# terry19850829Home/kafkastreams-cep

Hardware: AMD Instinct MI355X
Metric: events/sec (whole node), 3-stage A->B->C over 1M keys; achieved HBM GB/s (higher is better)
Workload: dtype int32; 1 GPU; C2: 3-stage strict A->B->C, processor mode; events_per_gpu=100000000, keys_per_gpu=1000000, matches_per_gpu=1531088, matches_total=1531088, parallelism=1 GPU, kernels=built-in, nfa_kernel=auto

## Files before the change

kafkastreams-cep_amd/csrc/compile.cpp:

```cpp
#include <math.h>
#include <string.h>

#include <algorithm>
#include <limits>

#include "kcep_internal.h"
#include "../../include/kcep.h"

namespace kcep {
namespace {

struct Reader {
  const uint8_t* p;
  size_t n, i = 0;
  bool bad = false;
  bool need(size_t k) {
    if (i + k > n) bad = true;
    return !bad;
  }
  template <class T>
  T get() {
    T v{};
    if (need(sizeof(T))) { memcpy(&v, p + i, sizeof(T)); i += sizeof(T); }
    return v;
// ... 335 lines not shown
  if (S.coltype == T_I32) {
    for (auto& b : bi) b = std::max<int64_t>(b, INT32_MIN);
    bi.erase(std::remove_if(bi.begin(), bi.end(), [](int64_t b) { return b > INT32_MAX; }), bi.end());
  }
  for (auto& b : tb) b = std::max<int64_t>(b, INT32_MIN);
  tb.erase(std::remove_if(tb.begin(), tb.end(), [](int64_t b) { return b > INT32_MAX; }), tb.end());
  uniq(bi); uniq(bf); uniq(tb);
  const int nb = int(isf ? bf.size() : bi.size());
  if (nb > 15 || tb.size() > 3) return false;
  S.nbp = nb;
  S.ntbp = int(tb.size());
  for (int i = 0; i < nb; i++) { if (isf) S.bpf[i] = bf[i]; else S.bpi[i] = bi[i]; }
  for (size_t i = 0; i < tb.size(); i++) S.tbp[i] = int32_t(tb[i]);
  memset(S.table, 0, sizeof S.table);
  memset(S.nan_mask, 0, sizeof S.nan_mask);
  for (int it = 0; it <= S.ntbp; it++) {
    const int64_t trep = it == 0 ? (S.ntbp ? int64_t(S.tbp[0]) - 1 : 0) : int64_t(S.tbp[it - 1]);
    for (int iv = 0; iv <= nb; iv++) {
      int64_t vi = 0;
      double vf = 0;
      if (isf) vf = iv == 0 ? -INFINITY : bf[iv - 1];
      else vi = iv == 0 ? (nb ? bi[0] - (bi[0] > IMIN ? 1 : 0) : 0) : bi[iv - 1];
      uint8_t m = 0;
      for (int s = 0; s < STENCIL_MAX_K; s++) m |= uint8_t(stage_accepts(S, s, isf, vi, vf, trep)) << s;
      S.table[it * 16 + iv] = m;
    }
    uint8_t m = 0;
    for (int s = 0; s < STENCIL_MAX_K; s++) m |= uint8_t(stage_accepts(S, s, isf, 0, NAN, trep)) << s;
    S.nan_mask[it] = m;
  }
  S.lut_n = 0;
  S.lut_lo = 0;
  memset(S.lut, 0, sizeof S.lut);
  if (!isf && S.ntbp == 0 && nb >= 6 && bi.back() - bi.front() < int64_t(sizeof S.lut)) {
    S.lut_lo = bi.front();
    S.lut_n = int32_t(bi.back() - bi.front() + 1);
    for (int r = 0, iv = 0; r < S.lut_n; r++) {
      while (iv < nb && bi[iv] <= S.lut_lo + r) iv++;
      S.lut[r] = S.table[iv];
    }
  }
  return true;
}

bool stencil_shape(const Program& P, uint32_t& opt, std::string& why) {
  auto no = [&](const char* w) { why = w; return false; };
  const int k = int(P.pats.size());
  if (k > STENCIL_MAX_K) return no("more than 8 stages");
  opt = 0;
  for (int i = 0; i < k; i++) {
    const auto& p = P.pats[i];
    if (p.strategy != S_STRICT) return no("non-strict selection strategy");
    if (p.one_or_more || p.times > 1) return no("quantifier");
    if (p.optional) {
      if (i == 0) return no("optional first stage");
      opt |= 1u << i;
    }
    if (!p.folds.empty()) return no("fold");
    for (int j = 0; j < i; j++)
      if (P.pats[j].name_id == p.name_id) return no("duplicate stage names");
  }
  if (opt && k > CHAIN_MAX_K) return no("optional stages in a pattern of more than 4 stages");
  return true;
}

void put_slot(StencilProgram& S, int slot, const DNF& d) {
  S.nterms[slot] = int(d.size());
  S.pslots |= 1 << slot;
  for (size_t t = 0; t < d.size(); t++) {
    const Term& tm = d[t];
    S.vi[slot][t] = tm.has_v ? StencilAtomI{tm.v.lo, tm.v.hi} : StencilAtomI{IMIN, IMAX};
    S.vf[slot][t] = tm.has_v ? StencilAtomF{tm.v.dlo, tm.v.dhi} : StencilAtomF{-INFINITY, INFINITY};
    S.tp[slot][t] = tm.has_t ? StencilAtomI{tm.t.lo, tm.t.hi} : StencilAtomI{IMIN, IMAX};
// ... 344 lines not shown
  memset(&M, 0, sizeof M);
  CodeGen cg;
  cg.names = &P.names;
  const char* unfit = nullptr;
  auto slot = [&](int s, const ExprP& pred) {
    if (!unfit) unfit = mask_unfit(pred);
    if (unfit || !event_only(pred)) return;
    mask_reads(pred, M);
    M.pslots |= 1 << s;
    M.pc[s] = cg.emit(pred);
  };
  for (int i = 0; i < k; i++) {
    const auto& p = P.pats[i];
    S.name[i] = p.name_id;
    slot(i, p.topic >= 0 ? mk(OP_AND, mk_topic(p.topic), p.pred) : p.pred);
    if (opt >> i & 1) slot(CHAIN_MAX_K + i, P.pats[i + 1].pred);
  }
  if (unfit) return no(unfit);
  if (!cg.ok) return no(cg.why);
  if (cg.maxdepth > NFA_STACK) return no("expression nests deeper than the device operand stack");
  if (cg.code.size() > size_t(NFA_MAX_CODE)) return no("predicate code too large");
  M.ncols = int32_t(P.coltypes.size());
  for (size_t c = 0; c < P.coltypes.size(); c++) M.coltype[c] = P.coltypes[c];
  M.ncode = int32_t(cg.code.size());
  memcpy(M.code, cg.code.data(), cg.code.size() * sizeof(int32_t));
  S.k = k;
  S.chain = opt ? 1 : 0;
  S.optmask = int32_t(opt);
  S.pslots = M.pslots;
  S.col = -1;
  S.coltype = T_I32;
  S.lut_lo = 0;
  S.lut_n = 256;
  for (int m = 0; m < 256; m++) S.lut[m] = uint8_t(m);
  P.mask_ok = true;
  P.mask_why.clear();
}

}

int lower_general(Program& P, std::string& why) {
  DevProgram& D = P.dev;
  memset(&D, 0, sizeof D);
  if (P.stages.size() > size_t(NFA_MAX_STAGES)) { why = "too many stages"; return CEP_E_UNSUPPORTED; }
  if (P.states.size() > size_t(NFA_MAX_STATES)) { why = "too many states"; return CEP_E_UNSUPPORTED; }
  if (P.coltypes.size() > 16) { why = "too many columns"; return CEP_E_UNSUPPORTED; }
  D.nstages = int32_t(P.stages.size());
  D.begin = P.begin;
  D.nstates = int32_t(P.states.size());
  D.ncols = int32_t(P.coltypes.size());
  {
    std::vector<int> depth(P.stages.size(), 1);
    for (int id = 0; id < int(P.stages.size()); id++)
      for (auto& e : P.stages[id].edges)
        if ((e.op == E_PROCEED || e.op == E_SKIP_PROCEED) && e.target >= 0)
          depth[id] = std::max(depth[id], depth[e.target] + 1);
    int m = 0;
    for (int d : depth) m = std::max(m, d);
    D.maxdepth = m + 1;
    if (D.maxdepth > NFA_MAX_FRAMES) { why = "PROCEED chain deeper than the device frame stack"; return CEP_E_UNSUPPORTED; }
  }
  for (size_t c = 0; c < P.coltypes.size(); c++) D.coltype[c] = P.coltypes[c];
  D.ndefined = int32_t(P.defined_states.size());
  for (size_t i = 0; i < P.defined_states.size(); i++) D.defined[i] = P.defined_states[i];
  std::vector<std::pair<int, int>> slots;
  CodeGen cg;
  cg.names = &P.names;
// ... 132 lines not shown
```

kafkastreams-cep_amd/csrc/follow.hip:

```cpp
#include "stencil_kernel.h"

namespace kcep {

static_assert(FOLLOW_TILE == ST_TILE, "follow_bits takes the stencil kernels' tile: one chunk per thread");
static_assert(FOLLOW_TILE == 64 * 64, "a tile is 64 bitmap words: one second-level word");

typedef unsigned long long u64;

int64_t follow_tiles(int64_t n) { return (std::max<int64_t>(n, 1) + FOLLOW_TILE - 1) / FOLLOW_TILE; }

struct FollowMaps {
  const u64* bits;
  const u64* sum;
  int64_t wpl;
  int64_t nt;
  int64_t n;
  int32_t k;
  uint32_t next;
};

__device__ __forceinline__ int64_t next_set(const u64* __restrict__ plane, const u64* __restrict__ sum, int64_t from,
                                            int64_t limit) {
  if (from >= limit) return limit;
  int64_t w = from >> 6;
// ... 8 lines not shown
    sx = sum[sw];
  }
  w = sw * 64 + __builtin_ctzll(sx);
  return w * 64 + __builtin_ctzll(plane[w]);
}

__device__ __forceinline__ int64_t follow_walk(const FollowMaps& M, int64_t j0, int32_t* __restrict__ row) {
  const int64_t E = next_set(M.bits + M.k * M.wpl, M.sum + M.k * M.nt, j0 + 1, M.n);
  const int64_t end = E < M.n ? E : M.n;
  int64_t p = j0;
  if (row) row[0] = int32_t(j0);
  for (int s = 1; s < M.k; s++) {
    const u64* plane = M.bits + s * M.wpl;
    p++;
    if (M.next >> s & 1) {
      p = next_set(plane, M.sum + s * M.nt, p, end);
      if (p >= end) return -1;
    } else if (p >= end || !(plane[p >> 6] >> (p & 63) & 1)) {
      return -1;
    }
    if (row) row[s] = int32_t(p);
  }
  return p;
}

template <class VT, bool TOPIC>
__global__ __launch_bounds__(ST_THREADS) void follow_bits(const int32_t* __restrict__ key, const VT* __restrict__ val,
                                                         const int32_t* __restrict__ topic, int64_t n,
                                                         const StencilProgram* __restrict__ P, int k,
                                                         u64* __restrict__ bits, u64* __restrict__ sum, int64_t wpl,
                                                         int64_t nt, int64_t* __restrict__ tile_starts) {
  __shared__ __attribute__((aligned(16))) uint8_t s_mask[ST_TILE];
  __shared__ __attribute__((aligned(16))) uint8_t s_ks[ST_TILE];
  __shared__ uint8_t s_tab[64];
  __shared__ uint8_t s_lut[256];
  __shared__ uint8_t s_nan[4];
  __shared__ uint32_t s_part[STENCIL_MAX_K + 1][ST_THREADS / 64];
  __shared__ int32_t s_cnt[ST_THREADS / 64];

  const int tid = threadIdx.x;
  const int lane = tid & 63, wid = tid >> 6;
  if (tid < 64) s_tab[tid] = P->table[tid];
  s_lut[tid] = P->lut[tid];
  if (tid < 4) s_nan[tid] = P->nan_mask[tid];
  const int64_t tile = blockIdx.x;
  const int64_t base = tile * ST_TILE;

  Chunk<VT, TOPIC> cur;
  load_chunk<VT, TOPIC>(cur, key, val, topic, base, n, tid);
  int32_t before[ST_EPT / 4];
#pragma unroll
  for (int q = 0; q < ST_EPT / 4; q++) {
    const int64_t g = base + q * (ST_THREADS * 4) + tid * 4;
    before[q] = 0;
    if (lane == 0 && g > 0 && g < n) before[q] = key[g - 1];
  }
  __syncthreads();
  uint32_t packed[4];
  masks_of_chunk<VT, TOPIC>(cur, P, s_tab, s_nan, packed, s_lut);
#pragma unroll
  for (int q = 0; q < ST_EPT / 4; q++) {
    const int local = q * (ST_THREADS * 4) + tid * 4;
    const int64_t g = base + local;
    const v4i kv = cur.k[q];
    int32_t kp = __shfl_up(kv[3], 1);
    if (lane == 0) kp = before[q];
    uint32_t ks = uint32_t(g == 0 || kp != kv[0]) | (uint32_t(kv[1] != kv[0]) << 8) | (uint32_t(kv[2] != kv[1]) << 16) |
                  (uint32_t(kv[3] != kv[2]) << 24);
    uint32_t w = packed[q];
    const int64_t left = n - g;
    if (left < 4) {
      const uint32_t keep = left <= 0 ? 0u : (0xFFFFFFFFu >> (8 * (4 - left)));
      w &= keep;
      ks &= keep;
    }
    *reinterpret_cast<uint32_t*>(&s_mask[local]) = w;
    *reinterpret_cast<uint32_t*>(&s_ks[local]) = ks;
  }
  __syncthreads();
  u64 mine[STENCIL_MAX_K + 1];
#pragma unroll
  for (int s = 0; s <= STENCIL_MAX_K; s++) mine[s] = 0;
  for (int i = 0; i < 16; i++) {
    const int r = (wid * 16 + i) * 64 + lane;
    const uint32_t m = s_mask[r];
    const u64 bk = __ballot(s_ks[r] != 0);
    if (lane == i) mine[STENCIL_MAX_K] = bk;
#pragma unroll
    for (int s = 0; s < STENCIL_MAX_K; s++) {
      if (s < k) {
        const u64 bs = __ballot((m >> s & 1) != 0);
        if (lane == i) mine[s] = bs;
// ... 126 lines not shown
```

kafkastreams-cep_amd/csrc/kcep_internal.h:

```cpp
#pragma once
#include <hip/hip_runtime_api.h>
#include <stdint.h>
#include "kcep_dev.h"

#include <memory>
#include <string>
#include <vector>

namespace kcep {

struct Expr {
  uint8_t op = 0, t = 0, ct = 0;
  int32_t i32 = 0;
  int64_t i64 = 0;
  double f64 = 0;
  int col = 0, name = 0;
  std::string sname;
  std::shared_ptr<Expr> a, b;
};
using ExprP = std::shared_ptr<Expr>;

struct Fold {
  int state;
  uint8_t type;
// ... 4 lines not shown
  std::string name;
  int name_id = 0, level = 0;
  uint8_t strategy = S_STRICT;
  int32_t topic = -1;
  uint8_t one_or_more = 0, optional = 0;
  int32_t times = 1;
  int64_t window_ms = -1;
  ExprP pred;
  std::vector<Fold> folds;
};

struct EdgeDef {
  uint8_t op;
  ExprP pred;
  int target;
};

struct StageDef {
  int id, name;
  uint8_t type;
  int64_t window_ms;
  int pattern;
  std::vector<EdgeDef> edges;
};

constexpr int STENCIL_MAX_K = 8;
constexpr int STENCIL_MAX_TERMS = 6;
constexpr int STENCIL_MAX_ATOMS = 2;

struct StencilAtomI { int64_t lo, hi; };
struct StencilAtomF { double lo, hi; };

constexpr int CHAIN_MAX_K = 4;
struct StencilProgram {
  int32_t k;
  int32_t col;
  int32_t coltype;
  int32_t use_topic;
  int32_t chain;
  int32_t optmask;
  int32_t pslots;
  int32_t nterms[STENCIL_MAX_K];
  int32_t hasv[STENCIL_MAX_K][STENCIL_MAX_TERMS];
  StencilAtomI vi[STENCIL_MAX_K][STENCIL_MAX_TERMS];
  StencilAtomF vf[STENCIL_MAX_K][STENCIL_MAX_TERMS];
  StencilAtomI tp[STENCIL_MAX_K][STENCIL_MAX_TERMS];
  int32_t name[STENCIL_MAX_K];
  int32_t nbp;
  int32_t ntbp;
  int64_t bpi[15];
  double bpf[15];
  int32_t tbp[3];
  uint8_t table[64];
  uint8_t nan_mask[4];
  int64_t lut_lo;
  int32_t lut_n;
  uint8_t lut[256];
};

struct Program {
  std::vector<uint8_t> coltypes;
  std::vector<PatternDef> pats;
  std::vector<StageDef> stages;
  std::vector<std::string> names;
  std::vector<std::string> states;
  std::vector<int> defined_states;
  int begin = -1;
  bool general_ok = false;
  std::string general_why;
  DevProgram dev{};
  bool stencil_ok = false;
  std::string stencil_why;
  bool runs_ok = false;
  bool has_seq = false;
  std::string runs_why;
  StencilProgram stencil{};
  bool mask_ok = false;
  std::string mask_why;
  StencilProgram mask_stencil{};
  MaskProgram mask_prog{};
  bool follow_ok = false;
  std::string follow_why;
  StencilProgram follow{};
  uint32_t follow_next = 0;
};

struct HaloHdr {
  int32_t stamp[2];
  int32_t claim;
  uint8_t cnt[2];
// ... 27 lines not shown
```

kafkastreams-cep_amd/csrc/stencil_kernel.h:

```cpp
#pragma once
#include <hip/hip_runtime.h>
#include <stdint.h>

#include <type_traits>

#include "launch.h"

namespace kcep {

constexpr int ST_THREADS = 256;
constexpr int ST_EPT = 16;
constexpr int ST_TILE = ST_THREADS * ST_EPT;
constexpr int ST_SUB = 4;
inline int stencil_sub(int64_t ntiles) { return ntiles >= int64_t(ST_SUB) * 2048 ? ST_SUB : 1; }

typedef int v4i __attribute__((ext_vector_type(4)));
typedef long long v2l __attribute__((ext_vector_type(2)));
__device__ __forceinline__ v4i ld_nt4(const void* p) { return __builtin_nontemporal_load(reinterpret_cast<const v4i*>(p)); }
__device__ __forceinline__ v2l ld_nt2(const void* p) { return __builtin_nontemporal_load(reinterpret_cast<const v2l*>(p)); }

__device__ __forceinline__ int kpos(int rp) { return rp + 4 * (rp >> 4); }
constexpr int ST_KWORDS = (ST_TILE + 16) + 4 * ((ST_TILE + 16) >> 4) + 16;

template <class VT>
// ... 31 lines not shown
  for (int q = 0; q < ST_EPT / 4; q++) {
    const int64_t g = base + q * STRIDE + tid * 4;
    if (g + 3 < n) {
      if constexpr (KEYS) c.k[q] = ld_nt4(key + g);
      if constexpr (sizeof(VT) == 4) {
        c.v[q].a = ld_nt4(val + g);
      } else {
        c.v[q].a = ld_nt2(val + g);
        c.v[q].b = ld_nt2(val + g + 2);
      }
      if constexpr (TOPIC) c.t[q] = ld_nt4(topic + g);
    } else {
      const int64_t g0 = g < n ? g : n - 1, g1 = g + 1 < n ? g + 1 : n - 1;
      const int64_t g2 = g + 2 < n ? g + 2 : n - 1, g3 = g + 3 < n ? g + 3 : n - 1;
      if constexpr (KEYS) c.k[q] = v4i{key[g0], key[g1], key[g2], key[g3]};
      if constexpr (sizeof(VT) == 4) {
        c.v[q].a = v4i{__builtin_bit_cast(int32_t, val[g0]), __builtin_bit_cast(int32_t, val[g1]),
                       __builtin_bit_cast(int32_t, val[g2]), __builtin_bit_cast(int32_t, val[g3])};
      } else {
        c.v[q].a = v2l{__builtin_bit_cast(long long, val[g0]), __builtin_bit_cast(long long, val[g1])};
        c.v[q].b = v2l{__builtin_bit_cast(long long, val[g2]), __builtin_bit_cast(long long, val[g3])};
      }
      if constexpr (TOPIC) c.t[q] = v4i{topic[g0], topic[g1], topic[g2], topic[g3]};
    }
  }
}

template <class VT>
__device__ __forceinline__ VT bp_at(const StencilProgram* __restrict__ P, int b) {
  if constexpr (std::is_same<VT, double>::value) return P->bpf[b];
  else return VT(P->bpi[b]);
}

template <class VT, bool TOPIC>
__device__ __forceinline__ void masks_of_chunk(const Chunk<VT, TOPIC>& c, const StencilProgram* __restrict__ P,
                                               const uint8_t* s_tab, const uint8_t* s_nan, uint32_t (&packed)[4],
                                               const uint8_t* s_lut) {
  if constexpr (!TOPIC && !std::is_same<VT, double>::value) {
    const int32_t lut_n = P->lut_n;
    if (lut_n > 0) {
      const int64_t lo = P->lut_lo;
      const uint32_t below = s_tab[0], above = s_tab[P->nbp];
#pragma unroll
      for (int q = 0; q < 4; q++) {
        uint32_t w = 0;
#pragma unroll
        for (int i = 0; i < 4; i++) {
          const int64_t dv = int64_t(vget<VT>(c.v[q], i)) - lo;
          const uint32_t m = dv < 0 ? below : dv >= lut_n ? above : uint32_t(s_lut[dv]);
          w |= m << (8 * i);
        }
        packed[q] = w;
      }
      return;
    }
  }
  int iv[ST_EPT], it[ST_EPT];
#pragma unroll
  for (int e = 0; e < ST_EPT; e++) { iv[e] = 0; it[e] = 0; }
  const int nbp = P->nbp;
  for (int b = 0; b < nbp; b++) {
    const VT bp = bp_at<VT>(P, b);
#pragma unroll
    for (int e = 0; e < ST_EPT; e++) iv[e] += bp <= vget<VT>(c.v[e >> 2], e & 3) ? 1 : 0;
  }
  if constexpr (TOPIC) {
    const int ntbp = P->ntbp;
    for (int b = 0; b < ntbp; b++) {
      const int32_t tb = P->tbp[b];
#pragma unroll
      for (int e = 0; e < ST_EPT; e++) {
        const int32_t tv = c.t[e >> 2][e & 3];
        it[e] += tb <= tv ? 1 : 0;
      }
    }
  }
#pragma unroll
  for (int q = 0; q < 4; q++) {
    uint32_t w = 0;
#pragma unroll
    for (int i = 0; i < 4; i++) {
      const int e = 4 * q + i;
      uint32_t m = s_tab[it[e] * 16 + iv[e]];
      if constexpr (std::is_same<VT, double>::value) {
        const double v = vget<VT>(c.v[q], i);
        if (v != v) m = s_nan[it[e]];
      }
      w |= m << (8 * i);
    }
    packed[q] = w;
  }
}

template <class VT, bool TOPIC>
__device__ __forceinline__ uint32_t mask_of(const StencilProgram* __restrict__ P, const uint8_t* s_tab,
                                            const uint8_t* s_nan, VT v, int32_t t, const uint8_t* s_lut) {
  if constexpr (!TOPIC && !std::is_same<VT, double>::value) {
    const int32_t lut_n = P->lut_n;
    if (lut_n > 0) {
      const int64_t dv = int64_t(v) - P->lut_lo;
      return dv < 0 ? s_tab[0] : dv >= lut_n ? s_tab[P->nbp] : s_lut[dv];
    }
  }
  int iv = 0, it = 0;
  for (int b = 0; b < P->nbp; b++) iv += bp_at<VT>(P, b) <= v ? 1 : 0;
  if constexpr (TOPIC)
    for (int b = 0; b < P->ntbp; b++) it += P->tbp[b] <= t ? 1 : 0;
  if constexpr (std::is_same<VT, double>::value)
    if (v != v) return s_nan[it];
  return s_tab[it * 16 + iv];
}

template <int K>
struct ChainWin {
  uint32_t b[K];
  uint32_t s[K];
  uint32_t same;
};

__device__ __forceinline__ uint32_t byte_bits(uint64_t m, int i) {
  return uint32_t((((m >> i) & 0x0101010101010101ull) * 0x0102040810204080ull) >> 56);
}

template <int K>
__device__ __forceinline__ ChainWin<K> chain_window(const int32_t (&wk)[24], const uint64_t (&m8)[3], uint32_t opt) {
  ChainWin<K> c;
#pragma unroll
  for (int i = 0; i < K; i++) { c.b[i] = 0; c.s[i] = 0; }
  c.same = 0;
#pragma unroll
  for (int q = 0; q < 3; q++) {
#pragma unroll
    for (int i = 0; i < K; i++) {
      c.b[i] |= byte_bits(m8[q], i) << (8 * q);
      c.s[i] |= byte_bits(m8[q], CHAIN_MAX_K + i) << (8 * q);
    }
  }
#pragma unroll
  for (int w = 1; w < 24; w++) c.same |= uint32_t(wk[w] == wk[w - 1]) << w;
#pragma unroll
  for (int i = 0; i < K; i++)
    if (!((opt >> i) & 1)) c.s[i] = 0;
  return c;
// ... 119 lines not shown
        if ((m >> stage) & 1) { cm |= 1u << stage; stage++; alive = true; break; }
        if (((opt >> stage) & 1) && ((m >> (CHAIN_MAX_K + stage)) & 1)) { stage++; continue; }
        break;
      }
      if (!alive) break;
      if (stage == K) { done = v == d; break; }
    }
    if (done) { res |= 1u << d; cms[d] = cm; }
  }
  return res;
}

__device__ __forceinline__ int32_t stencil_row(int32_t rj, uint32_t a, int s, int k, bool chain, bool carry) {
  if (chain) {
    const uint32_t d = a & 3u, cm = (a >> 2) & 15u;
    const int ho = int(a >> 6);
    const int rel = -int32_t(d) + __popc(cm & ((1u << s) - 1));
    if (!((cm >> s) & 1)) return -1;
    if (carry && ho != 3 && rel < -ho) return -(1 + (-ho - rel));
    return rj + rel;
  }
  const int need = carry ? int(a) : 0;
  return s < need ? -(1 + (need - s)) : rj - (k - 1) + s;
}

template <int K, class VT, bool TOPIC, bool CHAIN, bool CARRY, int SUB>
__global__ __launch_bounds__(ST_THREADS) void stencil_kernel(
    const int32_t* __restrict__ key, const VT* __restrict__ val, const int32_t* __restrict__ topic, int64_t n,
    const StencilProgram* __restrict__ P, int32_t* __restrict__ out, int64_t* __restrict__ tile_count,
    int64_t ntiles, StencilCarry C) {
  __shared__ __attribute__((aligned(16))) int32_t s_key[ST_KWORDS];
  __shared__ __attribute__((aligned(16))) uint8_t s_mask[ST_TILE + 16];
  __shared__ int32_t s_wsum[SUB][ST_THREADS / 64];
  __shared__ uint8_t s_tab[64];
  __shared__ uint8_t s_lut[256];
  __shared__ uint8_t s_nan[4];
  __shared__ uint32_t s_super;

  const int tid = threadIdx.x;
  const int lane = tid & 63, wid = tid >> 6;
  if (tid == 0) s_super = blockIdx.x;
  if (tid < 64) s_tab[tid] = P->table[tid];
  s_lut[tid] = P->lut[tid];
  if (tid < 4) s_nan[tid] = P->nan_mask[tid];
  __syncthreads();
  const int64_t tile0 = int64_t(s_super) * SUB;
  const int ntl = int(ntiles - tile0 < SUB ? ntiles - tile0 : SUB);

  Chunk<VT, TOPIC> cur;
  load_chunk<VT, TOPIC>(cur, key, val, topic, tile0 * ST_TILE, n, tid);
  int32_t h_key = INT32_MIN;
  uint32_t h_mask = 0;
  VT h_val{};
  int32_t h_top = 0;
  const bool halo_lane = tid >= 16 - (K - 1) && tid < 16;
  const bool h_first = halo_lane && tile0 * ST_TILE - 16 + tid >= 0;
  if (h_first) {
    const int64_t g = tile0 * ST_TILE - 16 + tid;
    h_key = key[g];
    h_val = val[g];
    if constexpr (TOPIC) h_top = topic[g];
  }

  uint32_t hits[SUB];
  uint64_t bneed[CARRY ? SUB : 1];
  int excl[SUB], total[SUB];
  uint32_t wpk[CHAIN ? SUB : 1][2 * K], wsame[CHAIN ? SUB : 1];
  uint32_t hb[CHAIN && CARRY ? SUB : 1];
  const uint32_t opt = CHAIN ? uint32_t(P->optmask) : 0u;

#pragma unroll
  for (int j = 0; j < SUB; j++) {
    hits[j] = 0; excl[j] = 0; total[j] = 0;
    if (j < ntl) {
      const int64_t tile = tile0 + j;
      const int64_t base = tile * ST_TILE;
      const int lb = ST_EPT * tid + 8;
// ... 16 lines not shown
        ck[24] = tid + 1 < ST_THREADS ? s_key[kpos(lb + 24)] : (base + ST_TILE < n ? key[base + ST_TILE] : INT32_MIN);
        const int64_t g0 = base + tid * ST_EPT;
        uint32_t starts = 0;
#pragma unroll
        for (int i = 0; i < ST_EPT; i++) {
          const int32_t kj = ck[8 + i];
          bool full = true;
#pragma unroll
          for (int t = 1; t < K; t++) full = full && ck[8 + i - t] == kj;
          const bool live = g0 + i < n;
          bnd |= uint32_t(live && !full) << i;
          endm |= uint32_t(live && (ck[9 + i] != kj || g0 + i + 1 >= n)) << i;
          starts |= uint32_t(ck[7 + i] != kj) << i;
        }
        starts &= bnd;
        todo = bnd | endm;
        if (todo) {
          ka = ck[8 + __ffs(todo) - 1];
          kb = ck[8 + 31 - __clz(todo)];
          oka = key_ok(C, ka);
          okb = kb != ka && key_ok(C, kb);
          ra = halo_load(C, oka ? ka : 0);
          rb = halo_load(C, okb ? kb : 0);
          if (C.grouped) starts = 0;
          while (starts) {
            const int i = __ffs(starts) - 1;
            starts &= starts - 1;
            const int32_t ks = s_key[kpos(lb + 8 + i)];
            if (ks >= 0 && ks < C.max_keys) twice |= atomicMax(&C.hdr[ks].claim, C.stamp) == C.stamp;
          }
        }
      }
      uint32_t packed[4];
      masks_of_chunk<VT, TOPIC>(cur, P, s_tab, s_nan, packed, s_lut);
#pragma unroll
      for (int q = 0; q < ST_EPT / 4; q++) {
        const int local = q * (ST_THREADS * 4) + tid * 4;
        uint32_t w = packed[q];
        const int64_t left = n - (base + local);
        if (left < 4) w &= left <= 0 ? 0u : (0xFFFFFFFFu >> (8 * (4 - left)));
        if constexpr (!CARRY) *reinterpret_cast<v4i*>(&s_key[kpos(16 + local)]) = cur.k[q];
        *reinterpret_cast<uint32_t*>(&s_mask[16 + local]) = w;
      }
      if (tid < 16) {
        if (j == 0 && h_first) h_mask = mask_of<VT, TOPIC>(P, s_tab, s_nan, h_val, h_top, s_lut);
        if constexpr (!CARRY) s_key[kpos(tid)] = halo_lane ? h_key : INT32_MIN;
        s_mask[tid] = halo_lane ? uint8_t(h_mask) : 0;
      }
      __syncthreads();
      if (j + 1 < ntl) load_chunk<VT, TOPIC>(cur, key, val, topic, base + ST_TILE, n, tid);

      int32_t wk[24];
      uint8_t wm[24];
      uint64_t m8s[3];
#pragma unroll
      for (int q = 0; q < 6; q++) {
        const v4i k4 = *reinterpret_cast<const v4i*>(&s_key[kpos(lb + 4 * q)]);
        wk[4 * q] = k4[0]; wk[4 * q + 1] = k4[1]; wk[4 * q + 2] = k4[2]; wk[4 * q + 3] = k4[3];
      }
#pragma unroll
      for (int q = 0; q < 3; q++) {
        const uint64_t m8 = *reinterpret_cast<const uint64_t*>(&s_mask[lb + 8 * q]);
        m8s[q] = m8;
#pragma unroll
        for (int b = 0; b < 8; b++) wm[8 * q + b] = uint8_t(m8 >> (8 * b));
      }
      uint32_t hit = 0;
      int cnt = 0;
      if constexpr (CHAIN) {
        const ChainWin<K> cw = chain_window<K>(wk, m8s, opt);
        ChainEnds<K> ce;
        ce.run(cw, 0, 0, nullptr);
#pragma unroll
        for (int d = 1; d < K; d++) cnt += __popc(ce.e[d] & 0xFFFF00u);
#pragma unroll
        for (int i = 0; i < K; i++) { wpk[j][i] = cw.b[i]; wpk[j][K + i] = cw.s[i]; }
        wsame[j] = cw.same;
      } else {
// ... 168 lines not shown
      }
      mbase += total[j];
    }
  }
}



template <class VT, bool TOPIC, bool KEYS = true>
__device__ __forceinline__ void load_tile(Chunk<VT, TOPIC>& c, const int32_t* __restrict__ key,
                                          const VT* __restrict__ val, const int32_t* __restrict__ topic,
                                          int64_t base, int64_t n, int tid) {
  if (base + ST_TILE > n) {
    load_chunk<VT, TOPIC, ST_THREADS * 4, KEYS>(c, key, val, topic, base, n, tid);
    return;
  }
  const int32_t* kb = key + base;
  const VT* vb = val + base;
  const int32_t* tb = TOPIC ? topic + base : nullptr;
#pragma unroll
  for (int q = 0; q < ST_EPT / 4; q++) {
    const uint32_t o = uint32_t(q * (ST_THREADS * 4) + tid * 4);
    if constexpr (KEYS) c.k[q] = ld_nt4(kb + o);
    if constexpr (sizeof(VT) == 4) {
      c.v[q].a = ld_nt4(vb + o);
    } else {
      c.v[q].a = ld_nt2(vb + o);
      c.v[q].b = ld_nt2(vb + o + 2);
    }
    if constexpr (TOPIC) c.t[q] = ld_nt4(tb + o);
  }
}

#ifndef ST_PLAIN_DENSE_LANES
#define ST_PLAIN_DENSE_LANES 40
#endif
constexpr int ST_KEYS_ADAPTIVE = 0, ST_KEYS_SPARSE = 1, ST_KEYS_DENSE = 2;
template <int K>
__device__ __forceinline__ uint32_t window_same_keys(const int32_t* __restrict__ key, int64_t g0, int64_t n,
                                                     uint32_t cand, int mode, int lane) {
  const uint64_t holders = __ballot(cand != 0);
  if (holders == 0) return 0;
  const bool dense = mode == ST_KEYS_DENSE || (mode == ST_KEYS_ADAPTIVE && __popcll(holders) > ST_PLAIN_DENSE_LANES);
  int32_t k[ST_EPT], pk[K - 1];
#pragma unroll
  for (int i = 0; i < ST_EPT; i++) k[i] = 0;
#pragma unroll
  for (int t = 0; t < K - 1; t++) pk[t] = 0;
  auto own = [&](bool nt) {
    if (g0 + ST_EPT <= n) {
#pragma unroll
      for (int q = 0; q < ST_EPT / 4; q++) {
        const v4i v = nt ? ld_nt4(key + g0 + 4 * q) : *reinterpret_cast<const v4i*>(key + g0 + 4 * q);
        k[4 * q] = v[0]; k[4 * q + 1] = v[1]; k[4 * q + 2] = v[2]; k[4 * q + 3] = v[3];
      }
    } else {
#pragma unroll
      for (int i = 0; i < ST_EPT; i++) k[i] = key[g0 + i < n ? g0 + i : n - 1];
    }
  };
  auto before = [&]() {
#pragma unroll
    for (int t = 0; t < K - 1; t++) {
      const int64_t g = g0 - (K - 1) + t;
      pk[t] = key[g < 0 ? 0 : g < n ? g : n - 1];
    }
// ... 4 lines not shown
    for (int t = 0; t < K - 1; t++)
      pk[t] = __builtin_amdgcn_update_dpp(0, k[ST_EPT - (K - 1) + t], 0x138, 0xF, 0xF, false);
    if (lane == 0) before();
  } else {
    if (cand != 0) own(false);
    if (cand & ((1u << (K - 1)) - 1u)) before();
  }
  uint32_t S = uint32_t(k[0] == pk[K - 2]) << 8;
#pragma unroll
  for (int i = 1; i < ST_EPT; i++) S |= uint32_t(k[i] == k[i - 1]) << (8 + i);
#pragma unroll
  for (int t = 1; t < K - 1; t++) S |= uint32_t(pk[t] == pk[t - 1]) << (8 - (K - 1) + t);
  return S;
}

#ifndef ST_PLAIN_WAVES
#define ST_PLAIN_WAVES 6
#endif
#ifndef ST_CARRY_WAVES
#define ST_CARRY_WAVES 4
#endif
template <int K, class VT, bool TOPIC, int SUB, bool CARRY>
__global__ __launch_bounds__(ST_THREADS, CARRY ? ST_CARRY_WAVES : ST_PLAIN_WAVES) void stencil_plain_kernel(
    const int32_t* __restrict__ key, const VT* __restrict__ val, const int32_t* __restrict__ topic, int64_t n,
    const StencilProgram* __restrict__ P, int32_t* __restrict__ out, int64_t* __restrict__ tile_count,
    int64_t ntiles, StencilCarry C, int key_mode, uint16_t* __restrict__ tile_count16) {
  static_assert(K >= 1 && K <= 7, "bit 7 of a record's byte is its same-key bit");
  static_assert(ST_SUB * ST_TILE <= 0xFFFF, "a super-tile's match count is also stored as a 16-bit word");
  __shared__ __attribute__((aligned(16))) uint8_t s_mask[ST_TILE + 16];
  __shared__ int32_t s_bk[CARRY ? ST_TILE + 16 : 1];
  __shared__ int32_t s_lastk[CARRY ? 2 : 1][CARRY ? 17 : 1];
  __shared__ int32_t s_firstk[CARRY ? 16 : 1];
  __shared__ int32_t s_wsum[2][ST_THREADS / 64];
  __shared__ uint8_t s_tab[64];
  __shared__ uint8_t s_lut[256];
  __shared__ uint8_t s_nan[4];
  __shared__ int32_t s_out[CARRY ? 1 : ST_TILE];

  const int tid = threadIdx.x;
  const int lane = tid & 63, wid = tid >> 6;
  if (tid < 64) s_tab[tid] = P->table[tid];
  s_lut[tid] = P->lut[tid];
  if (tid < 4) s_nan[tid] = P->nan_mask[tid];
  const int64_t tile0 = int64_t(blockIdx.x) * SUB;
  const int ntl = int(ntiles - tile0 < SUB ? ntiles - tile0 : SUB);

  Chunk<VT, TOPIC> cur;
  load_tile<VT, TOPIC, CARRY>(cur, key, val, topic, tile0 * ST_TILE, n, tid);
  const bool halo_lane = tid >= 16 - (K - 1) && tid < 16;
  const int64_t hg = tile0 * ST_TILE - 16 + tid;
  int32_t h_key = INT32_MIN, h_prev = INT32_MIN, h_top = 0;
  VT h_val{};
  if (halo_lane && hg >= 0) {
    h_val = val[hg];
    if constexpr (TOPIC) h_top = topic[hg];
    if constexpr (CARRY) {
      h_key = key[hg];
      if (hg > 0) h_prev = key[hg - 1];
    }
  }
  int32_t before0 = INT32_MIN;
  if constexpr (CARRY)
    if (tid == 0 && tile0 > 0) before0 = key[tile0 * ST_TILE - 1];
  __syncthreads();
  uint32_t h_mask = 0;
  if (halo_lane && hg >= 0)
    h_mask = mask_of<VT, TOPIC>(P, s_tab, s_nan, h_val, h_top, s_lut) | (uint32_t(CARRY && hg > 0 && h_prev == h_key) << 7);
  int32_t h_bk = h_key;
  bool twice = false;

  int32_t* slot = out + tile0 * int64_t(ST_TILE) * K;
  uint8_t* const aux = reinterpret_cast<uint8_t*>(slot + SUB * ST_TILE);
  int64_t sum = 0;
  int nbuf = 0;
  int32_t* const dense = out + int64_t(blockIdx.x) * ST_DENSE;
  int32_t* const over = out + int64_t(gridDim.x) * ST_DENSE + tile0 * ST_TILE;
  for (int j = 0; j < ntl; j++) {
    const int64_t base = (tile0 + j) * ST_TILE;
    int32_t nk = INT32_MIN;
    if constexpr (CARRY)
      if (tid == ST_THREADS - 1 && base + ST_TILE < n) nk = key[base + ST_TILE];
    uint32_t packed[4];
    masks_of_chunk<VT, TOPIC>(cur, P, s_tab, s_nan, packed, s_lut);
#pragma unroll
    for (int q = 0; q < ST_EPT / 4; q++) {
      const int local = q * (ST_THREADS * 4) + tid * 4;
      uint32_t w = packed[q];
      const int64_t left = n - (base + local);
      if constexpr (CARRY) {
        const v4i k = cur.k[q];
        const int32_t kp = __builtin_amdgcn_update_dpp(INT32_MIN, k[3], 0x138, 0xF, 0xF, false);
        const uint32_t same = uint32_t(lane > 0 && kp == k[0]) | (uint32_t(k[1] == k[0]) << 8) |
                              (uint32_t(k[2] == k[1]) << 16) | (uint32_t(k[3] == k[2]) << 24);
        w |= same << 7;
        if (lane == 0) s_firstk[4 * q + wid] = k[0];
        if (lane == 63) s_lastk[j & 1][4 * q + wid + 1] = k[3];
        const int32_t kn = __builtin_amdgcn_update_dpp(INT32_MIN, k[0], 0x130, 0xF, 0xF, false);
        const bool c1 = k[1] != k[0] || left <= 1, c2 = k[2] != k[1] || left <= 2, c3 = k[3] != k[2] || left <= 3;
        if (lane == 0 || kp != k[0] || c1) s_bk[16 + local] = k[0];
        if (c1 || c2) s_bk[16 + local + 1] = k[1];
        if (c2 || c3) s_bk[16 + local + 2] = k[2];
        if (c3 || lane == 63 || kn != k[3] || left <= 4) s_bk[16 + local + 3] = k[3];
      }
      if (left < 4) w &= left <= 0 ? 0u : (0xFFFFFFFFu >> (8 * (4 - left)));
      *reinterpret_cast<uint32_t*>(&s_mask[16 + local]) = w;
    }
    if (tid < 16) s_mask[tid] = halo_lane ? uint8_t(h_mask) : 0;
    if constexpr (CARRY)
      if (tid < 16) s_bk[tid] = h_bk;
    if constexpr (CARRY)
      if (j == 0 && tid == 0) s_lastk[0][0] = before0;
    if (j + 1 < ntl) load_tile<VT, TOPIC, CARRY>(cur, key, val, topic, base + ST_TILE, n, tid);
    __syncthreads();

    const int lb = ST_EPT * tid + 8;
    uint64_t m8[3];
#pragma unroll
    for (int q = 0; q < 3; q++) m8[q] = *reinterpret_cast<const uint64_t*>(&s_mask[lb + 8 * q]);
    uint32_t S = 0;
    if constexpr (CARRY) {
#pragma unroll
      for (int q = 0; q < 3; q++) S |= byte_bits(m8[q], 7) << (8 * q);
      const int rb = ((ST_EPT * tid + 15) >> 8) << 8;
      const int pb = rb - (ST_EPT * tid - 8);
      if (pb >= 0 && pb < 24) {
        const int m = rb >> 8;
        const int32_t kb = m == 0 ? (j == 0 ? s_lastk[0][0] : s_lastk[(j - 1) & 1][16]) : s_lastk[j & 1][m];
        S = (S & ~(1u << pb)) | (uint32_t(kb == s_firstk[m]) << pb);
      }
    }
    uint32_t h = 0xFFFFFFFFu;
    uint32_t Bs[K];
#pragma unroll
    for (int s = 0; s < K; s++) {
      uint32_t B = 0;
#pragma unroll
      for (int q = 0; q < 3; q++) B |= byte_bits(m8[q], s) << (8 * q);
      Bs[s] = B;
      h &= B << (K - 1 - s);
    }
    if constexpr (!CARRY && K > 1)
      S = window_same_keys<K>(key, base + ST_EPT * tid, n, (h >> 8) & 0xFFFFu, key_mode, lane);
#pragma unroll
    for (int d = 0; d < K - 1; d++) h &= S << d;
    uint32_t hit = (h >> 8) & 0xFFFFu;
    uint64_t bneed = 0;
    if constexpr (CARRY) {
      const int rn = ST_EPT * tid + 16;
      uint32_t sn = 0;
      if ((rn & 255) == 0) {
        const int m = rn >> 8;
        sn = m < 16 ? uint32_t(s_lastk[j & 1][m] == s_firstk[m]) : uint32_t(base + ST_TILE < n && nk == s_lastk[j & 1][16]);
      } else {
        sn = s_mask[16 + rn] >> 7;
      }
      const int64_t g0 = base + ST_EPT * tid;
      if (g0 + ST_EPT >= n) sn = 0;
      const int64_t left = n - g0;
      const uint32_t live = left >= 16 ? 0xFFFFu : left <= 0 ? 0u : (1u << left) - 1u;
      S &= (live << 8) | 0xFFu;
      const uint32_t Sown = (S >> 8) & 0xFFFFu;
      const uint32_t starts = ~Sown & live;
      const uint32_t ends = ~((S >> 9) | (sn << 15)) & live;
      uint32_t cand = 0;
#pragma unroll
      for (int o = 0; o < K - 1; o++) {
        uint32_t c = ~S << o;
#pragma unroll
        for (int t = 0; t < o; t++) c &= S << t;
#pragma unroll
        for (int t = 0; t <= o; t++) c &= Bs[K - 1 - o + t] << (o - t);
        cand |= c;
      }
      cand = (cand >> 8) & live;
      uint32_t todo = cand | ends | starts;
// ... 177 lines not shown
```

Measured before the change: 1052 billion events/s.

## Clamp LUT lookups with med3, batch breakpoints, and skip tail masking on whole tiles

The dense mask LUT gets sentinel entries at both ends, so a lookup becomes a single clamp (v_med3_i32) and index instead of two compare-selects, and the LUT now applies to int32 columns with as few as one breakpoint. Breakpoints are staged in a shared table and read uniformly in pairs. Tail masking is skipped when a tile is fully inside the input. The non-carry stencil computes window hits with a SWAR bit-gather instead of per-stage byte_bits loops. Together these cut ALU work in the mask and hit stages, at the cost of more template code and a changed LUT layout that the compiler and kernels must agree on.

```diff
diff --git a/kafkastreams-cep_amd/csrc/compile.cpp b/kafkastreams-cep_amd/csrc/compile.cpp
--- a/kafkastreams-cep_amd/csrc/compile.cpp
+++ b/kafkastreams-cep_amd/csrc/compile.cpp
@@ -391,13 +391,17 @@
   S.lut_n = 0;
   S.lut_lo = 0;
   memset(S.lut, 0, sizeof S.lut);
-  if (!isf && S.ntbp == 0 && nb >= 6 && bi.back() - bi.front() < int64_t(sizeof S.lut)) {
+  const int64_t tmin = S.coltype == T_I32 ? int64_t(INT32_MIN) : IMIN, tmax = S.coltype == T_I32 ? int64_t(INT32_MAX) : IMAX;
+  if (!isf && S.ntbp == 0 && nb >= (S.coltype == T_I32 ? 1 : 3) && uint64_t(bi.back()) - uint64_t(bi.front()) < uint64_t(STENCIL_LUT_MAX) &&
+      bi.front() > tmin && bi.back() < tmax) {
     S.lut_lo = bi.front();
     S.lut_n = int32_t(bi.back() - bi.front() + 1);
+    S.lut[0] = S.table[0];
     for (int r = 0, iv = 0; r < S.lut_n; r++) {
       while (iv < nb && bi[iv] <= S.lut_lo + r) iv++;
-      S.lut[r] = S.table[iv];
-    }
+      S.lut[1 + r] = S.table[iv];
+    }
+    S.lut[1 + S.lut_n] = S.table[nb];
   }
   return true;
 }
@@ -808,7 +812,7 @@
   S.coltype = T_I32;
   S.lut_lo = 0;
   S.lut_n = 256;
-  for (int m = 0; m < 256; m++) S.lut[m] = uint8_t(m);
+  for (int m = 0; m < 256; m++) S.lut[1 + m] = uint8_t(m);
   P.mask_ok = true;
   P.mask_why.clear();
 }
diff --git a/kafkastreams-cep_amd/csrc/follow.hip b/kafkastreams-cep_amd/csrc/follow.hip
--- a/kafkastreams-cep_amd/csrc/follow.hip
+++ b/kafkastreams-cep_amd/csrc/follow.hip
@@ -64,17 +64,14 @@
                                                          int64_t nt, int64_t* __restrict__ tile_starts) {
   __shared__ __attribute__((aligned(16))) uint8_t s_mask[ST_TILE];
   __shared__ __attribute__((aligned(16))) uint8_t s_ks[ST_TILE];
-  __shared__ uint8_t s_tab[64];
-  __shared__ uint8_t s_lut[256];
-  __shared__ uint8_t s_nan[4];
+  __shared__ MaskTables<VT> s_mt;
   __shared__ uint32_t s_part[STENCIL_MAX_K + 1][ST_THREADS / 64];
   __shared__ int32_t s_cnt[ST_THREADS / 64];
 
   const int tid = threadIdx.x;
   const int lane = tid & 63, wid = tid >> 6;
-  if (tid < 64) s_tab[tid] = P->table[tid];
-  s_lut[tid] = P->lut[tid];
-  if (tid < 4) s_nan[tid] = P->nan_mask[tid];
+  load_tables<VT>(s_mt, P, tid);
+  const MaskUni<VT> U = load_uni<VT>(P);
   const int64_t tile = blockIdx.x;
   const int64_t base = tile * ST_TILE;
 
@@ -89,7 +86,7 @@
   }
   __syncthreads();
   uint32_t packed[4];
-  masks_of_chunk<VT, TOPIC>(cur, P, s_tab, s_nan, packed, s_lut);
+  masks_of_chunk<VT, TOPIC>(cur, P, s_mt, U, packed);
 #pragma unroll
   for (int q = 0; q < ST_EPT / 4; q++) {
     const int local = q * (ST_THREADS * 4) + tid * 4;
diff --git a/kafkastreams-cep_amd/csrc/kcep_internal.h b/kafkastreams-cep_amd/csrc/kcep_internal.h
--- a/kafkastreams-cep_amd/csrc/kcep_internal.h
+++ b/kafkastreams-cep_amd/csrc/kcep_internal.h
@@ -60,6 +60,7 @@
 struct StencilAtomF { double lo, hi; };
 
 constexpr int CHAIN_MAX_K = 4;
+constexpr int STENCIL_LUT_MAX = 256;
 struct StencilProgram {
   int32_t k;
   int32_t col;
@@ -83,7 +84,7 @@
   uint8_t nan_mask[4];
   int64_t lut_lo;
   int32_t lut_n;
-  uint8_t lut[256];
+  uint8_t lut[STENCIL_LUT_MAX + 8];
 };
 
 struct Program {
diff --git a/kafkastreams-cep_amd/csrc/stencil_kernel.h b/kafkastreams-cep_amd/csrc/stencil_kernel.h
--- a/kafkastreams-cep_amd/csrc/stencil_kernel.h
+++ b/kafkastreams-cep_amd/csrc/stencil_kernel.h
@@ -87,41 +87,91 @@
   else return VT(P->bpi[b]);
 }
 
+constexpr int ST_BPG = 2;
+template <class VT>
+struct MaskTables {
+  uint8_t tab[64];
+  uint8_t lut[STENCIL_LUT_MAX + 8];
+  uint8_t nan[4];
+  __attribute__((aligned(16))) VT bp[16];
+};
+template <class VT>
+struct MaskUni {
+  int nbp, ntbp, lut_n;
+  VT lo1, hi;
+};
+
+template <class VT>
+__device__ __forceinline__ void load_tables(MaskTables<VT>& T, const StencilProgram* __restrict__ P, int tid) {
+  static_assert(ST_THREADS == STENCIL_LUT_MAX, "one dense-table entry per thread, the padding by the first 8");
+  if (tid < 64) T.tab[tid] = P->table[tid];
+  T.lut[tid] = P->lut[tid];
+  if (tid < 8) T.lut[STENCIL_LUT_MAX + tid] = P->lut[STENCIL_LUT_MAX + tid];
+  if (tid < 4) T.nan[tid] = P->nan_mask[tid];
+  if (tid < 16) T.bp[tid] = tid < 15 ? bp_at<VT>(P, tid) : VT(0);
+}
+template <class VT>
+__device__ __forceinline__ MaskUni<VT> load_uni(const StencilProgram* __restrict__ P) {
+  MaskUni<VT> U{P->nbp, P->ntbp, 0, VT(0), VT(0)};
+  if constexpr (!std::is_same<VT, double>::value) {
+    U.lut_n = P->lut_n;
+    U.lo1 = VT(P->lut_lo - 1);
+    U.hi = VT(P->lut_lo + P->lut_n);
+  }
+  return U;
+}
+
+template <class VT>
+__device__ __forceinline__ uint32_t lut_index(VT v, const MaskUni<VT>& U) {
+  if constexpr (sizeof(VT) == 4) {
+    int32_t c;
+    asm("v_med3_i32 %0, %1, %2, %3" : "=v"(c) : "v"(v), "s"(U.lo1), "v"(U.hi));
+    return uint32_t(c) - uint32_t(U.lo1);
+  } else {
+    const VT c = v < U.lo1 ? U.lo1 : v > U.hi ? U.hi : v;
+    return uint32_t(uint64_t(c)) - uint32_t(uint64_t(U.lo1));
+  }
+}
+
 template <class VT, bool TOPIC>
 __device__ __forceinline__ void masks_of_chunk(const Chunk<VT, TOPIC>& c, const StencilProgram* __restrict__ P,
-                                               const uint8_t* s_tab, const uint8_t* s_nan, uint32_t (&packed)[4],
-                                               const uint8_t* s_lut) {
+                                               const MaskTables<VT>& T, const MaskUni<VT>& U, uint32_t (&packed)[4]) {
   if constexpr (!TOPIC && !std::is_same<VT, double>::value) {
-    const int32_t lut_n = P->lut_n;
-    if (lut_n > 0) {
-      const int64_t lo = P->lut_lo;
-      const uint32_t below = s_tab[0], above = s_tab[P->nbp];
-#pragma unroll
-      for (int q = 0; q < 4; q++) {
-        uint32_t w = 0;
-#pragma unroll
-        for (int i = 0; i < 4; i++) {
-          const int64_t dv = int64_t(vget<VT>(c.v[q], i)) - lo;
-          const uint32_t m = dv < 0 ? below : dv >= lut_n ? above : uint32_t(s_lut[dv]);
-          w |= m << (8 * i);
-        }
-        packed[q] = w;
-      }
+    if (U.lut_n > 0) {
+      uint32_t m[ST_EPT];
+#pragma unroll
+      for (int e = 0; e < ST_EPT; e++) m[e] = T.lut[lut_index<VT>(vget<VT>(c.v[e >> 2], e & 3), U)];
+#pragma unroll
+      for (int q = 0; q < 4; q++) packed[q] = m[4 * q] | (m[4 * q + 1] << 8) | (m[4 * q + 2] << 16) | (m[4 * q + 3] << 24);
       return;
     }
   }
   int iv[ST_EPT], it[ST_EPT];
 #pragma unroll
   for (int e = 0; e < ST_EPT; e++) { iv[e] = 0; it[e] = 0; }
-  const int nbp = P->nbp;
-  for (int b = 0; b < nbp; b++) {
-    const VT bp = bp_at<VT>(P, b);
-#pragma unroll
-    for (int e = 0; e < ST_EPT; e++) iv[e] += bp <= vget<VT>(c.v[e >> 2], e & 3) ? 1 : 0;
+  for (int b = 0; b < U.nbp; b += ST_BPG) {
+    VT bp[ST_BPG];
+#pragma unroll
+    for (int u = 0; u < ST_BPG; u++) {
+      if constexpr (sizeof(VT) == 4) {
+        bp[u] = __builtin_amdgcn_readfirstlane(__builtin_bit_cast(int32_t, T.bp[b + u]));
+      } else {
+        const uint64_t x = __builtin_bit_cast(uint64_t, T.bp[b + u]);
+        const uint32_t lo = uint32_t(__builtin_amdgcn_readfirstlane(int32_t(uint32_t(x))));
+        const uint32_t hi = uint32_t(__builtin_amdgcn_readfirstlane(int32_t(uint32_t(x >> 32))));
+        bp[u] = __builtin_bit_cast(VT, (uint64_t(hi) << 32) | lo);
+      }
+    }
+#pragma unroll
+    for (int u = 0; u < ST_BPG; u++) {
+      if (b + u < U.nbp) {
+#pragma unroll
+        for (int e = 0; e < ST_EPT; e++) iv[e] += bp[u] <= vget<VT>(c.v[e >> 2], e & 3) ? 1 : 0;
+      }
+    }
   }
   if constexpr (TOPIC) {
-    const int ntbp = P->ntbp;
-    for (int b = 0; b < ntbp; b++) {
+    for (int b = 0; b < U.ntbp; b++) {
       const int32_t tb = P->tbp[b];
 #pragma unroll
       for (int e = 0; e < ST_EPT; e++) {
@@ -136,10 +186,10 @@
 #pragma unroll
     for (int i = 0; i < 4; i++) {
       const int e = 4 * q + i;
-      uint32_t m = s_tab[it[e] * 16 + iv[e]];
+      uint32_t m = T.tab[it[e] * 16 + iv[e]];
       if constexpr (std::is_same<VT, double>::value) {
         const double v = vget<VT>(c.v[q], i);
-        if (v != v) m = s_nan[it[e]];
+        if (v != v) m = T.nan[it[e]];
       }
       w |= m << (8 * i);
     }
@@ -148,22 +198,18 @@
 }
 
 template <class VT, bool TOPIC>
-__device__ __forceinline__ uint32_t mask_of(const StencilProgram* __restrict__ P, const uint8_t* s_tab,
-                                            const uint8_t* s_nan, VT v, int32_t t, const uint8_t* s_lut) {
+__device__ __forceinline__ uint32_t mask_of(const StencilProgram* __restrict__ P, const MaskTables<VT>& T,
+                                            const MaskUni<VT>& U, VT v, int32_t t) {
   if constexpr (!TOPIC && !std::is_same<VT, double>::value) {
-    const int32_t lut_n = P->lut_n;
-    if (lut_n > 0) {
-      const int64_t dv = int64_t(v) - P->lut_lo;
-      return dv < 0 ? s_tab[0] : dv >= lut_n ? s_tab[P->nbp] : s_lut[dv];
-    }
+    if (U.lut_n > 0) return T.lut[lut_index<VT>(v, U)];
   }
   int iv = 0, it = 0;
-  for (int b = 0; b < P->nbp; b++) iv += bp_at<VT>(P, b) <= v ? 1 : 0;
+  for (int b = 0; b < U.nbp; b++) iv += T.bp[b] <= v ? 1 : 0;
   if constexpr (TOPIC)
-    for (int b = 0; b < P->ntbp; b++) it += P->tbp[b] <= t ? 1 : 0;
+    for (int b = 0; b < U.ntbp; b++) it += P->tbp[b] <= t ? 1 : 0;
   if constexpr (std::is_same<VT, double>::value)
-    if (v != v) return s_nan[it];
-  return s_tab[it * 16 + iv];
+    if (v != v) return T.nan[it];
+  return T.tab[it * 16 + iv];
 }
 
 template <int K>
@@ -349,17 +395,14 @@
   __shared__ __attribute__((aligned(16))) int32_t s_key[ST_KWORDS];
   __shared__ __attribute__((aligned(16))) uint8_t s_mask[ST_TILE + 16];
   __shared__ int32_t s_wsum[SUB][ST_THREADS / 64];
-  __shared__ uint8_t s_tab[64];
-  __shared__ uint8_t s_lut[256];
-  __shared__ uint8_t s_nan[4];
+  __shared__ MaskTables<VT> s_mt;
   __shared__ uint32_t s_super;
 
   const int tid = threadIdx.x;
   const int lane = tid & 63, wid = tid >> 6;
   if (tid == 0) s_super = blockIdx.x;
-  if (tid < 64) s_tab[tid] = P->table[tid];
-  s_lut[tid] = P->lut[tid];
-  if (tid < 4) s_nan[tid] = P->nan_mask[tid];
+  load_tables<VT>(s_mt, P, tid);
+  const MaskUni<VT> U = load_uni<VT>(P);
   __syncthreads();
   const int64_t tile0 = int64_t(s_super) * SUB;
   const int ntl = int(ntiles - tile0 < SUB ? ntiles - tile0 : SUB);
@@ -442,18 +485,21 @@
         }
       }
       uint32_t packed[4];
-      masks_of_chunk<VT, TOPIC>(cur, P, s_tab, s_nan, packed, s_lut);
+      masks_of_chunk<VT, TOPIC>(cur, P, s_mt, U, packed);
+      const bool whole = base + ST_TILE <= n;
 #pragma unroll
       for (int q = 0; q < ST_EPT / 4; q++) {
         const int local = q * (ST_THREADS * 4) + tid * 4;
         uint32_t w = packed[q];
-        const int64_t left = n - (base + local);
-        if (left < 4) w &= left <= 0 ? 0u : (0xFFFFFFFFu >> (8 * (4 - left)));
+        if (!whole) {
+          const int64_t left = n - (base + local);
+          if (left < 4) w &= left <= 0 ? 0u : (0xFFFFFFFFu >> (8 * (4 - left)));
+        }
         if constexpr (!CARRY) *reinterpret_cast<v4i*>(&s_key[kpos(16 + local)]) = cur.k[q];
         *reinterpret_cast<uint32_t*>(&s_mask[16 + local]) = w;
       }
       if (tid < 16) {
-        if (j == 0 && h_first) h_mask = mask_of<VT, TOPIC>(P, s_tab, s_nan, h_val, h_top, s_lut);
+        if (j == 0 && h_first) h_mask = mask_of<VT, TOPIC>(P, s_mt, U, h_val, h_top);
         if constexpr (!CARRY) s_key[kpos(tid)] = halo_lane ? h_key : INT32_MIN;
         s_mask[tid] = halo_lane ? uint8_t(h_mask) : 0;
       }
@@ -688,6 +734,32 @@
   }
 }
 
+__device__ __forceinline__ uint32_t win_bits(const uint32_t (&w)[6], int D, int T) {
+  const int q = T >> 5, r = T & 31;
+  const uint32_t lo = w[D - 2 + q], hi = q < 2 ? w[D - 1 + q] : 0u;
+  return uint32_t(((uint64_t(hi) << 32) | lo) >> r);
+}
+__device__ __forceinline__ uint32_t lsb_gather(uint32_t x, uint32_t y) {
+  uint32_t z = (x & 0x01010101u) | ((y & 0x01010101u) << 4);
+  z |= z << 7;
+  z |= z << 14;
+  return (z >> 21) & 0xFFu;
+}
+template <int K>
+__device__ __forceinline__ uint32_t window_hits(const uint64_t (&m8)[3]) {
+  uint32_t w[6], a[4];
+#pragma unroll
+  for (int q = 0; q < 3; q++) { w[2 * q] = uint32_t(m8[q]); w[2 * q + 1] = uint32_t(m8[q] >> 32); }
+#pragma unroll
+  for (int D = 2; D < 6; D++) {
+    uint32_t acc = 0xFFFFFFFFu;
+#pragma unroll
+    for (int s = 0; s < K; s++) acc &= win_bits(w, D, 64 - 8 * (K - 1 - s) + s);
+    a[D - 2] = acc;
+  }
+  return lsb_gather(a[0], a[1]) | (lsb_gather(a[2], a[3]) << 8);
+}
+
 #ifndef ST_PLAIN_DENSE_LANES
 #define ST_PLAIN_DENSE_LANES 40
 #endif
@@ -758,16 +830,13 @@
   __shared__ int32_t s_lastk[CARRY ? 2 : 1][CARRY ? 17 : 1];
   __shared__ int32_t s_firstk[CARRY ? 16 : 1];
   __shared__ int32_t s_wsum[2][ST_THREADS / 64];
-  __shared__ uint8_t s_tab[64];
-  __shared__ uint8_t s_lut[256];
-  __shared__ uint8_t s_nan[4];
+  __shared__ MaskTables<VT> s_mt;
   __shared__ int32_t s_out[CARRY ? 1 : ST_TILE];
 
   const int tid = threadIdx.x;
   const int lane = tid & 63, wid = tid >> 6;
-  if (tid < 64) s_tab[tid] = P->table[tid];
-  s_lut[tid] = P->lut[tid];
-  if (tid < 4) s_nan[tid] = P->nan_mask[tid];
+  load_tables<VT>(s_mt, P, tid);
+  const MaskUni<VT> U = load_uni<VT>(P);
   const int64_t tile0 = int64_t(blockIdx.x) * SUB;
   const int ntl = int(ntiles - tile0 < SUB ? ntiles - tile0 : SUB);
 
@@ -791,7 +860,7 @@
   __syncthreads();
   uint32_t h_mask = 0;
   if (halo_lane && hg >= 0)
-    h_mask = mask_of<VT, TOPIC>(P, s_tab, s_nan, h_val, h_top, s_lut) | (uint32_t(CARRY && hg > 0 && h_prev == h_key) << 7);
+    h_mask = mask_of<VT, TOPIC>(P, s_mt, U, h_val, h_top) | (uint32_t(CARRY && hg > 0 && h_prev == h_key) << 7);
   int32_t h_bk = h_key;
   bool twice = false;
 
@@ -807,30 +876,35 @@
     if constexpr (CARRY)
       if (tid == ST_THREADS - 1 && base + ST_TILE < n) nk = key[base + ST_TILE];
     uint32_t packed[4];
-    masks_of_chunk<VT, TOPIC>(cur, P, s_tab, s_nan, packed, s_lut);
-#pragma unroll
-    for (int q = 0; q < ST_EPT / 4; q++) {
-      const int local = q * (ST_THREADS * 4) + tid * 4;
-      uint32_t w = packed[q];
-      const int64_t left = n - (base + local);
-      if constexpr (CARRY) {
-        const v4i k = cur.k[q];
-        const int32_t kp = __builtin_amdgcn_update_dpp(INT32_MIN, k[3], 0x138, 0xF, 0xF, false);
-        const uint32_t same = uint32_t(lane > 0 && kp == k[0]) | (uint32_t(k[1] == k[0]) << 8) |
-                              (uint32_t(k[2] == k[1]) << 16) | (uint32_t(k[3] == k[2]) << 24);
-        w |= same << 7;
-        if (lane == 0) s_firstk[4 * q + wid] = k[0];
-        if (lane == 63) s_lastk[j & 1][4 * q + wid + 1] = k[3];
-        const int32_t kn = __builtin_amdgcn_update_dpp(INT32_MIN, k[0], 0x130, 0xF, 0xF, false);
-        const bool c1 = k[1] != k[0] || left <= 1, c2 = k[2] != k[1] || left <= 2, c3 = k[3] != k[2] || left <= 3;
-        if (lane == 0 || kp != k[0] || c1) s_bk[16 + local] = k[0];
-        if (c1 || c2) s_bk[16 + local + 1] = k[1];
-        if (c2 || c3) s_bk[16 + local + 2] = k[2];
-        if (c3 || lane == 63 || kn != k[3] || left <= 4) s_bk[16 + local + 3] = k[3];
-      }
-      if (left < 4) w &= left <= 0 ? 0u : (0xFFFFFFFFu >> (8 * (4 - left)));
-      *reinterpret_cast<uint32_t*>(&s_mask[16 + local]) = w;
-    }
+    masks_of_chunk<VT, TOPIC>(cur, P, s_mt, U, packed);
+    auto image = [&](auto whole) {
+#pragma unroll
+      for (int q = 0; q < ST_EPT / 4; q++) {
+        const int local = q * (ST_THREADS * 4) + tid * 4;
+        uint32_t w = packed[q];
+        const int64_t left = decltype(whole)::value ? int64_t(8) : n - (base + local);
+        if constexpr (CARRY) {
+          const v4i k = cur.k[q];
+          const int32_t kp = __builtin_amdgcn_update_dpp(INT32_MIN, k[3], 0x138, 0xF, 0xF, false);
+          const uint32_t same = uint32_t(lane > 0 && kp == k[0]) | (uint32_t(k[1] == k[0]) << 8) |
+                                (uint32_t(k[2] == k[1]) << 16) | (uint32_t(k[3] == k[2]) << 24);
+          w |= same << 7;
+          if (lane == 0) s_firstk[4 * q + wid] = k[0];
+          if (lane == 63) s_lastk[j & 1][4 * q + wid + 1] = k[3];
+          const int32_t kn = __builtin_amdgcn_update_dpp(INT32_MIN, k[0], 0x130, 0xF, 0xF, false);
+          const bool c1 = k[1] != k[0] || left <= 1, c2 = k[2] != k[1] || left <= 2, c3 = k[3] != k[2] || left <= 3;
+          if (lane == 0 || kp != k[0] || c1) s_bk[16 + local] = k[0];
+          if (c1 || c2) s_bk[16 + local + 1] = k[1];
+          if (c2 || c3) s_bk[16 + local + 2] = k[2];
+          if (c3 || lane == 63 || kn != k[3] || left <= 4) s_bk[16 + local + 3] = k[3];
+        }
+        if constexpr (!decltype(whole)::value)
+          if (left < 4) w &= left <= 0 ? 0u : (0xFFFFFFFFu >> (8 * (4 - left)));
+        *reinterpret_cast<uint32_t*>(&s_mask[16 + local]) = w;
+      }
+    };
+    if (CARRY ? base + ST_TILE < n : base + ST_TILE <= n) image(std::true_type{});
+    else image(std::false_type{});
     if (tid < 16) s_mask[tid] = halo_lane ? uint8_t(h_mask) : 0;
     if constexpr (CARRY)
       if (tid < 16) s_bk[tid] = h_bk;
@@ -856,17 +930,20 @@
       }
     }
     uint32_t h = 0xFFFFFFFFu;
-    uint32_t Bs[K];
-#pragma unroll
-    for (int s = 0; s < K; s++) {
-      uint32_t B = 0;
-#pragma unroll
-      for (int q = 0; q < 3; q++) B |= byte_bits(m8[q], s) << (8 * q);
-      Bs[s] = B;
-      h &= B << (K - 1 - s);
-    }
-    if constexpr (!CARRY && K > 1)
-      S = window_same_keys<K>(key, base + ST_EPT * tid, n, (h >> 8) & 0xFFFFu, key_mode, lane);
+    uint32_t Bs[CARRY ? K : 1];
+    if constexpr (CARRY) {
+#pragma unroll
+      for (int s = 0; s < K; s++) {
+        uint32_t B = 0;
+#pragma unroll
+        for (int q = 0; q < 3; q++) B |= byte_bits(m8[q], s) << (8 * q);
+        Bs[s] = B;
+        h &= B << (K - 1 - s);
+      }
+    } else {
+      h = window_hits<K>(m8) << 8;
+      if constexpr (K > 1) S = window_same_keys<K>(key, base + ST_EPT * tid, n, h >> 8, key_mode, lane);
+    }
 #pragma unroll
     for (int d = 0; d < K - 1; d++) h &= S << d;
     uint32_t hit = (h >> 8) & 0xFFFFu;
```

After: 1092 billion events/s (median of 6 runs). 1.04x the previous value.
